# kevinh-e/BetaOne

Hardware: AMD Instinct MI355X
Metric: mcts_nodes_per_sec (higher is better)
Workload: dtype f32 (3 x f16 split, f32 accumulate)

## Files before the change

betaone_amd/csrc/bo_engine.cpp:

```cpp
#include "../../include/betaone_engine.h"
#include "../../include/betaone_lab.h"

#include "bo_tree.h"
#include "bo_fastw.h"
#include "bo_info.h"
#include "bo_select_wide.h"
#include "bo_replay.h"
#include "bo_train.h"
#include "bo_metrics.h"
#include "bo_pgn.h"
#include "bo_san.h"
#include "bo_analyse.h"
#include "bo_reanalyse.h"
#include "bo_perft.h"
#include "bo_mate.h"
#include "bo_anchor.h"
#include "bo_book.h"
#include "bo_merge.h"
#include "bo_tb.h"
#include "bo_nn_fused.h"
#include "bo_conv.h"
#include "bo_tower.h"
#include "bo_tower_wg.h"
#include "bo_tower_h.h"
// ... 546 lines not shown
    return BO_OK;
}
extern "C" int bo_step(bo_engine *e, const float *policy_dev, const float *value_dev, int policy_kind, float *nn_in_dev,
                       void *stream) {
    if (!e || !nn_in_dev) return fail(BO_E_ARG, "null argument");
    if (policy_kind != BO_POLICY_NONE && (!policy_dev || !value_dev)) return fail(BO_E_ARG, "policy/value required");
    return step_launch(e, policy_dev, value_dev, policy_kind, nn_in_dev, stream, StepTail{nullptr, nullptr, nullptr, nullptr, 0});
}
extern "C" int bo_step_heads(bo_engine *e, const float *logits_dev, const float *vpart_dev, const float *b1_dev, const float *w2_dev,
                             const float *b2_dev, int rows, float *nn_in_dev, void *stream) {
    if (!e || !nn_in_dev || !logits_dev || !vpart_dev || !b1_dev || !w2_dev || !b2_dev) return fail(BO_E_ARG, "null argument");
    if (e->fast) return fail(BO_E_CONFIG, "bo_step_heads: the reference-semantics search only (fast mode evaluates rows, not games)");
    if (rows < e->d.c.G) return fail(BO_E_ARG, "bo_step_heads: the partial sums must hold a row per game (rows >= G)");
    return step_launch(e, logits_dev, nullptr, BO_POLICY_LOGITS, nn_in_dev, stream, StepTail{vpart_dev, b1_dev, w2_dev, b2_dev, rows});
}

extern "C" int bo_search_poll(bo_engine *e, int32_t *n_running, int32_t *n_requested, int32_t *requested_mask, void *stream) {
    if (!e) return fail(BO_E_ARG, "null engine");
    const size_t G = (size_t)e->d.c.G;
    RT(rt_d2h(e->h_info, e->d_info_blk, 2 * G * 4, stream));
    const int *ph = e->h_info, *rq = e->h_info + G;
    RT(rt_sync(stream));
    int run = 0, req = 0;
    for (size_t g = 0; g < G; g++) {
        bool r = ph[g] == PH_RUN;
        bool q = r && rq[g] >= 0;
        run += r; req += q;
        if (requested_mask) requested_mask[g] = q ? 1 : 0;
    }
    if (n_running) *n_running = run;
// ... 2148 lines not shown
#else
    if (!stream) return BO_OK;
    RT((int)hipStreamDestroy((hipStream_t)stream));
    return BO_OK;
#endif
}

extern "C" int bo_nn_heads(const void *p_dev, const void *v_dev, const float *wp_dev, const float *bp_dev, const float *w1_dev,
                           const float *b1_dev, const float *w2_dev, const float *b2_dev, float *policy_out_dev, float *value_out_dev,
                           float *scratch_dev, int batch, int flags, void *stream) {
#if defined(BO_WAVE_EMU)
    (void)p_dev; (void)v_dev; (void)wp_dev; (void)bp_dev; (void)w1_dev; (void)b1_dev; (void)w2_dev; (void)b2_dev; (void)policy_out_dev;
    (void)value_out_dev; (void)scratch_dev; (void)batch; (void)flags; (void)stream;
    return fail(BO_E_CONFIG, "bo_nn_heads is a gfx950-only kernel");
#else
    if (!p_dev || !v_dev || !wp_dev || !bp_dev || !w1_dev || !b1_dev || !w2_dev || !b2_dev || !policy_out_dev || (!value_out_dev && !(flags & 4)) || !scratch_dev)
        return fail(BO_E_ARG, "null argument");
    if ((flags & 4) && (flags & 1)) return fail(BO_E_ARG, "bo_nn_heads: flags 4 (no rows kernel) leaves LOGITS: it excludes flags 1 (softmax)");
    if (batch < 1 || batch > 65536) return fail(BO_E_ARG, "bo_nn_heads: 1 <= batch <= 65536");
    bo_heads_args a;
    a.p = p_dev; a.v = v_dev; a.wp = wp_dev; a.bp = bp_dev; a.w1 = w1_dev; a.b1 = b1_dev; a.w2 = w2_dev; a.b2 = b2_dev;
    a.policy_out = policy_out_dev; a.value_out = value_out_dev;
    a.vpart = scratch_dev;
    a.B = batch; a.softmax = flags & 1; a.pb = bo_heads_policy_boards(batch);
    const int otw = 4 / (a.pb >> 5);
    const unsigned tiles = (unsigned)(((batch + a.pb - 1) / a.pb) * ((BO_HEADS_NA / 32 + otw - 1) / otw) + ((batch + 63) / 64) * 4 * BO_HEADS_KS);
    if (flags & 2) hipLaunchKernelGGL(bo_k_heads_tiles<true>, dim3(tiles), dim3(256), 0, (hipStream_t)stream, a, bo_heads_pair{});
    else hipLaunchKernelGGL(bo_k_heads_tiles<false>, dim3(tiles), dim3(256), 0, (hipStream_t)stream, a, bo_heads_pair{});
    if (!(flags & 4)) hipLaunchKernelGGL(bo_k_heads_rows, dim3((unsigned)batch), dim3(256), 0, (hipStream_t)stream, a);
    RT((int)hipGetLastError());
// ... 1170 lines not shown
```

betaone_amd/csrc/bo_heads.h:

```cpp
#pragma once
#if !defined(BO_WAVE_EMU)
#include <hip/hip_runtime.h>
#include "bo_tower.h"

#define BO_HEADS_NA 4672
#define BO_HEADS_KP 128
#define BO_HEADS_KV 2048
#define BO_HEADS_NH 256
#define BO_HEADS_KS 16
#define BO_HEADS_PITCH 132

struct bo_heads_args {
    const void *p, *v;
    const float *wp, *bp, *w1, *b1, *w2, *b2;
    float *policy_out, *value_out;
    float *vpart;
    int B, softmax;
    int pb;
};
static inline int bo_heads_policy_boards(int batch) { return batch > 64 ? 128 : batch > 32 ? 64 : 32; }

struct bo_heads_pair {
    const int32_t *sel = nullptr;
    const float *wp = nullptr, *bp = nullptr, *w1 = nullptr, *b1 = nullptr, *w2 = nullptr, *b2 = nullptr;
// ... 124 lines not shown
#pragma unroll
                        for (int rt = 0; rt < 2; rt++) acc[c][rt] = __builtin_amdgcn_mfma_f32_16x16x4f32(fw[c][e], fv[rt][e], acc[c][rt], 0, 0, 0);
            }
#pragma unroll
            for (int c = 0; c < 2; c++)
#pragma unroll
                for (int rt = 0; rt < 2; rt++) {
                    const int row = r0 + bb + 16 * rt + i;
                    if (row < B && (only_net < 0 || (pr.sel[row] != 0) == only_net))
                        *reinterpret_cast<bo_f32x4 *>(a.vpart + ((size_t)ks * B + row) * BO_HEADS_NH + h0 + hb + 16 * c + 4 * kq) = acc[c][rt];
                }
        }
    }
}

template <bool PAIR>
__device__ __forceinline__ void bo_heads_rows_body(const bo_heads_args &a, const bo_heads_pair &q) {
    __shared__ float sred[8];
    const int tid = threadIdx.x, lane = tid & 63, wave = __builtin_amdgcn_readfirstlane(tid >> 6);
    const int B = a.B, row = (int)blockIdx.x;
    const float *b1 = a.b1, *w2 = a.w2, *b2 = a.b2;
    if constexpr (PAIR) {
        if (__builtin_amdgcn_readfirstlane(q.sel[row]) != 0) { b1 = q.b1; w2 = q.w2; b2 = q.b2; }
    }
    float part[BO_HEADS_KS];
#pragma unroll
    for (int ks = 0; ks < BO_HEADS_KS; ks++) part[ks] = a.vpart[((size_t)ks * B + row) * BO_HEADS_NH + tid];
    bo_f32x4 *r4 = reinterpret_cast<bo_f32x4 *>(a.policy_out + (size_t)row * BO_HEADS_NA);
    constexpr int N4 = BO_HEADS_NA / 4, IT = (N4 + 255) / 256;
    const float ninf = -__builtin_inff();
    bo_f32x4 x[IT];
    float mx = ninf;
    if (a.softmax) {
#pragma unroll
        for (int u = 0; u < IT; u++) {
            const int k = tid + 256 * u;
            x[u] = k < N4 ? r4[k] : bo_f32x4{ninf, ninf, ninf, ninf};
        }
    }
    float hsum = 0.0f;
#pragma unroll
    for (int ks = 0; ks < BO_HEADS_KS; ks++) hsum += part[ks];
    hsum += b1[tid];
    hsum = (hsum > 0.0f ? hsum : 0.0f) * w2[tid];
    if (a.softmax) {
#pragma unroll
        for (int u = 0; u < IT; u++) mx = fmaxf(mx, fmaxf(fmaxf(x[u][0], x[u][1]), fmaxf(x[u][2], x[u][3])));
    }
#pragma unroll
    for (int m = 32; m >= 1; m >>= 1) { mx = fmaxf(mx, __shfl_xor(mx, m, 64)); hsum += __shfl_xor(hsum, m, 64); }
    if (lane == 0) { sred[wave] = mx; sred[4 + wave] = hsum; }
    __syncthreads();
    mx = fmaxf(fmaxf(sred[0], sred[1]), fmaxf(sred[2], sred[3]));
    if (tid == 0) a.value_out[row] = tanhf(((sred[4] + sred[5]) + (sred[6] + sred[7])) + b2[0]);
    if (a.softmax) {
        float sum = 0.0f;
#pragma unroll
        for (int u = 0; u < IT; u++) {
            if (tid + 256 * u < N4) {
#pragma unroll
                for (int e = 0; e < 4; e++) { x[u][e] = expf(x[u][e] - mx); sum += x[u][e]; }
            }
        }
#pragma unroll
        for (int m = 32; m >= 1; m >>= 1) sum += __shfl_xor(sum, m, 64);
        __syncthreads();
        if (lane == 0) sred[wave] = sum;
        __syncthreads();
        sum = (sred[0] + sred[1]) + (sred[2] + sred[3]);
#pragma unroll
        for (int u = 0; u < IT; u++) {
            const int k = tid + 256 * u;
            if (k < N4) r4[k] = bo_f32x4{x[u][0] / sum, x[u][1] / sum, x[u][2] / sum, x[u][3] / sum};
        }
    }
}

extern "C" __global__ void __launch_bounds__(256)
bo_k_heads_rows(bo_heads_args a) { bo_heads_rows_body<false>(a, bo_heads_pair{}); }

extern "C" __global__ void __launch_bounds__(256)
bo_k_heads_rows_pair(bo_heads_args a, bo_heads_pair q) { bo_heads_rows_body<true>(a, q); }

typedef _Float16 bo_hh8 __attribute__((ext_vector_type(8)));

#ifndef BO_HEADS_NT_STORES
#define BO_HEADS_NT_STORES 1
#endif
#define BO_HEADS_PS 10
#define BO_HEADS_PT 15
#define BO_HEADS_WPITCH (BO_HEADS_KP + 8)

struct bo_heads_h_args {
    const _Float16 *p, *v;
    const _Float16 *wp, *w1;
    const float *bp, *b1, *w2, *b2;
    float *policy_out, *value_out;
// ... 214 lines not shown
```

betaone_amd/csrc/bo_tree.h:

```cpp
#pragma once
#include "bo_chess.h"
#include "bo_tb_probe.h"
#include <math.h>

#define BO_CH_CAP 32
#define BO_PATH_CAP 1024
#define BO_RES_CAP 256
#define BO_PLANES 120
#ifndef BO_PROF_SLOTS
#define BO_PROF_SLOTS 16
#endif
#define BO_ROW (BO_PLANES * 64)

enum { PH_IDLE = 0, PH_RUN = 1, PH_DONE = 2 };
enum { ST_OK = 0, ST_NODE_OVERFLOW = 1, ST_DEPTH_OVERFLOW = 2, ST_NAN_SCORE = 4, ST_PLY_OVERFLOW = 8,
       ST_ILLEGAL_ACTION = 16, ST_UL_OVERFLOW = 32, ST_TRK_OVERFLOW = 64 };
enum { POLICY_NONE = 0, POLICY_LOGITS = 1, POLICY_PROBS = 2 };

struct EngCfg {
    int G, S, B;
    int NCAP, PLY_CAP, TRK_CAP;
    int nstride;
    int UL_MAX, CH_MAX;
    float cpuct, keep;
// ... 626 lines not shown
    if (bo_finite(x)) return x;
    *bad = true;
    return 0.0f;
}

struct StepShared {
    bo_mv moves[BO_MAX_MOVES];
    bo_mv moves2[BO_MAX_MOVES];
    float pv[BO_MAX_MOVES];
    int path[BO_PATH_CAP];
    int path2[BO_PATH_CAP];
    int bpath[8];
    float probs[BO_NUM_ACTIONS];
    int rank_of[2 * BO_CH_CAP];
    ChainBuf chain;
};

BO_DEV void load_probs(const float *row, int kind, float *out) {
    const int lane = bo_lane();
    if (kind == POLICY_PROBS) {
        for (int i = lane; i < BO_NUM_ACTIONS; i += 64) out[i] = row[i];
    } else {
        float mx, sum;
        bo_f4 v[BO_ROW_IT];
        row_load_max_sum(row, v, &mx, &sum);
        BO_UNROLL
        for (int i = 0; i < BO_ROW_IT; i++) {
            const int k = lane + 64 * i;
            if (k < BO_ROW_N4) {
                out[4 * k] = bo_exp_row(v[i].x - mx) / sum; out[4 * k + 1] = bo_exp_row(v[i].y - mx) / sum;
                out[4 * k + 2] = bo_exp_row(v[i].z - mx) / sum; out[4 * k + 3] = bo_exp_row(v[i].w - mx) / sum;
            }
        }
    }
    bo_sync();
}

BO_DEV void apply_root(const Eng &e, int g, const float *row, int kind, StepShared &sh, int *n_nodes_io, int *flags) {
    const size_t no = NOFF(e, g);
    const int lane = bo_lane();
    const int n = e.root_nlegal[g];
    const bo_mv *mv = e.root_moves + (size_t)g * BO_MAX_MOVES;
    load_probs(row, kind, sh.probs);
    int m = e.c.root_m < n ? e.c.root_m : n;
    if (m > BO_CH_CAP) m = BO_CH_CAP;
    bool bad = false;
    for (int j = lane; j < n; j += 64) sh.pv[j] = finite_or_zero(sh.probs[move_to_index(mv[j])], &bad);
    if (lane < 2 * BO_CH_CAP) sh.rank_of[lane] = -1;
    bo_sync();
    for (int j = lane; j < n; j += 64) {
        int r = stable_rank(sh.pv, n, j);
        if (r < m) sh.rank_of[r] = j;
    }
    bo_sync();
    const DPos P = e.npos[no];
    int nch = m;
    if (lane < m) {
        int j = sh.rank_of[lane];
// ... 56 lines not shown
    BO_UNROLL
    for (int w = 0; w < 4; w++) {
        float h = 0.0f;
        BO_UNROLL
        for (int ks = 0; ks < 16; ks++) h += r.part[w][ks];
        h += r.b1[w];
        s[w] = (h > 0.0f ? h : 0.0f) * r.w2[w];
    }
    for (int m = 32; m >= 1; m >>= 1) {
        BO_UNROLL
        for (int w = 0; w < 4; w++) s[w] = s[w] + bo_shfl_xor_f(s[w], m);
    }
    return tanhf(((s[0] + s[1]) + (s[2] + s[3])) + r.b2);
}

BO_DEV void apply_leaf(const Eng &e, int g, int leaf, const float *row, int kind, const float *value_of, const StepTail &vt, StepShared &sh,
                       int *n_ul_io, int *flags) {
    const size_t no = NOFF(e, g);
    const int lane = bo_lane();
    const int n = e.req_nlegal[g];
    const bo_mv *mv = e.req_moves + (size_t)g * BO_MAX_MOVES;
    int slot = *n_ul_io;
    if (slot >= e.c.UL_MAX) { *flags |= ST_UL_OVERFLOW; slot = e.c.UL_MAX - 1; }
    const size_t uo = (size_t)g * e.c.UL_MAX + slot;
    float value;
    bool bad = false;
    if (kind == POLICY_PROBS) {
        value = value_of[g];
        for (int j = lane; j < n; j += 64) sh.pv[j] = finite_or_zero(row[move_to_index(mv[j])], &bad);
    } else {
        float mx, sum;
        if (vt.vpart) {
            TailRegs tr;
            tail_load(vt, g, tr);
            row_max_sum(row, &mx, &sum);
            value = tail_value(tr);
        } else {
            value = value_of[g];
            row_max_sum(row, &mx, &sum);
        }
        for (int j = lane; j < n; j += 64) sh.pv[j] = finite_or_zero(bo_exp_row(row[move_to_index(mv[j])] - mx) / sum, &bad);
    }
// ... 8 lines not shown
    if (lane == 0) {
        e.ul_node[uo] = leaf;
        e.ul_nlegal[uo] = n;
        e.ul_value[uo] = value;
        e.eval_slot[no + leaf] = (short)slot;
    }
    *n_ul_io = slot + 1;
    bo_sync();
}


BO_DEV float tb_leaf_value(int t, int kc) {
    const float m = 1.0f - (float)kc * (1.0f / 1024.0f);
    return t == TERM_TB_LOSS ? m : t == TERM_TB_WIN ? -m : 0.0f;
}
template <bool TB>
BO_DEV int step_body(const Eng &e, int g, const float *policy, const float *value, int kind, float *nn_in, StepShared &sh, const StepTail &vt) {
    const int lane = bo_lane();
    const size_t no = NOFF(e, g);
    int flags = 0;
    int sims = e.sims_done[g], rows = e.rows[g], n_runs = e.n_runs[g], n_ul = e.n_ul[g], n_nodes = e.n_nodes[g];
    int req = e.req_node[g];
    int *rl = e.run_leaf + (size_t)g * e.c.B, *rc = e.run_cnt + (size_t)g * e.c.B;
    float *row = nn_in + (size_t)g * BO_ROW;

    const bool prof = e.c.profile != 0;
    unsigned long long pc[8] = {0, 0, 0, 0, 0, 0, 0, 0};
    int n_iter = 0, n_first = 0, n_burst = 0, n_burst_sims = 0, n_general = 0, n_swaps = 0;
    unsigned long long tk = prof ? bo_clock() : 0ull;
    const unsigned long long t_start = tk;
#define BO_PROF(slot)                                                    \
    if (prof) { const unsigned long long _n = bo_clock(); pc[slot] += _n - tk; tk = _n; }
    if (req >= 0 && kind == POLICY_NONE) return n_nodes;
    const float *lut = e.sqrt_lut;
    if (req >= 0) {
        if (req == 0) apply_root(e, g, policy + (size_t)g * BO_NUM_ACTIONS, kind, sh, &n_nodes, &flags);
        else apply_leaf(e, g, req, policy + (size_t)g * BO_NUM_ACTIONS, kind, value, vt, sh, &n_ul, &flags);
        req = -1;
    }
    BO_PROF(0)
    int phase = PH_RUN;
    bool burst_tables_staged = false;
    int term_budget = e.c.B;
    int b_depth = 0;
    float b_tv = 0.0f;
    int path_leaf = -1, path_depth = -1;
    for (;;) {
        if (sims >= e.c.S) {
            if (rows > 0) { flush_pending(e, g, n_runs, n_ul, &n_nodes, sh.path2, &flags, path_leaf, sh.path, path_depth); rows = n_runs = n_ul = 0; }
            BO_PROF(5)
            phase = PH_DONE;
            break;
// ... 102 lines not shown
    return n_nodes;
}
BO_KERNEL void bo_k_step(Eng e, const float *policy, const float *value, int kind, float *nn_in, StepTail vt) {
    BO_SHARED StepShared sh;
    const int g = bo_block();
    if (e.phase[g] != PH_RUN) return;
    step_body<false>(e, g, policy, value, kind, nn_in, sh, vt);
}
BO_KERNEL void bo_k_step_tb(Eng e, const float *policy, const float *value, int kind, float *nn_in, StepTail vt) {
    BO_SHARED StepShared sh;
    const int g = bo_block();
    if (e.phase[g] != PH_RUN) return;
    step_body<true>(e, g, policy, value, kind, nn_in, sh, vt);
}

BO_DEV int root_prepare(const Eng &e, int g, StepShared &sh) {
    const size_t no = NOFF(e, g);
    const int lane = bo_lane();
    const int ply = e.ply[g];
    const DPos P = e.gpos[(size_t)g * e.c.PLY_CAP + ply];
    if (lane == 0) {
        init_node(e, no, 0, -1, 1.0f, 0, P);
        e.n_nodes[g] = 1; e.sims_done[g] = 0; e.rows[g] = 0; e.n_runs[g] = 0; e.n_ul[g] = 0;
        e.req_node[g] = -1; e.phase[g] = PH_IDLE; e.root_nch[g] = 0;
        if (e.ctx_mode[g] == 0) {
            int nh = ply < 7 ? ply : 7;
            e.n_hist[g] = nh;
            for (int i = 0; i < nh; i++) e.hist[(size_t)g * 7 + i] = e.gpos[(size_t)g * e.c.PLY_CAP + ply - nh + i];
        }
    }
// ... 361 lines not shown
```

betaone_amd/csrc/bo_wave.h:

```cpp
#pragma once
#include <stdint.h>

#if defined(BO_WAVE_EMU)
#include "wave_emu.h"
#else
#include <hip/hip_runtime.h>
#define BO_DEV __device__ __forceinline__
#define BO_DEV_NOINLINE __device__ __noinline__
#define BO_KERNEL extern "C" __global__ __launch_bounds__(64)
#define BO_SHARED __shared__
#define BO_CONST_TABLE __device__ const

BO_DEV int bo_lane() { return (int)(threadIdx.x & 63u); }
BO_DEV int bo_block() { return (int)blockIdx.x; }
BO_DEV uint64_t bo_ballot(bool p) { return __ballot(p); }
BO_DEV void bo_sync() { __syncthreads(); }
BO_DEV int bo_shfl(int v, int src) { return __shfl(v, src, 64); }
BO_DEV int bo_shfl_xor(int v, int m) { return __shfl_xor(v, m, 64); }
BO_DEV int bo_shfl_up(int v, int d) { return __shfl_up(v, d, 64); }
BO_DEV int bo_atomic_add(int *p, int v) { return atomicAdd(p, v); }
BO_DEV int bo_atomic_or(int *p, int v) { return atomicOr(p, v); }
BO_DEV uint64_t bo_bitrev64(uint64_t x) { return __builtin_bitreverse64(x); }
BO_DEV unsigned long long bo_clock() { return (unsigned long long)clock64(); }
#define BO_ROW_XCHG(v, kind) \
    __builtin_amdgcn_update_dpp(0, (v), (kind) == 0 ? 0xB1 : (kind) == 1 ? 0x4E : (kind) == 2 ? 0x141 : 0x140, 0xF, 0xF, false)
#endif
#if !defined(BO_WAVE_EMU)
BO_DEV int bo_readlane(int v, int src) { return __builtin_amdgcn_readlane(v, __builtin_amdgcn_readfirstlane(src)); }
#else
static inline int bo_readlane(int v, int src) { return bo_shfl(v, src); }
#endif
// ... 66 lines not shown
```

betaone_amd/engine.py:

```python
from __future__ import annotations

import ctypes as C
import os
from typing import Dict, List, Optional, Sequence, Tuple

import numpy as np
import torch

NUM_ACTIONS = 4672
INPUT_CHANNELS = 120
ROW_FLOATS = 120 * 64
MAX_LEGAL = 256
RES_CAP = 256
POLICY_NONE, POLICY_LOGITS, POLICY_PROBS = 0, 1, 2

STATUS_BITS = {1: "node overflow", 2: "depth overflow", 4: "NaN or infinite evaluation (prior or value)", 8: "ply overflow",
               16: "illegal action", 32: "leaf cache overflow", 64: "tracker overflow", 128: "position range outside the array",
               256: "pi wider than the record's rows"}
ST_PLY_OVERFLOW, ST_ILLEGAL_ACTION = 8, 16
ST_PI_OVERFLOW = 256
ST_NODE_OVERFLOW = 1
ST_DEPTH_OVERFLOW = 2
ST_NAN_SCORE = 4

# ... 64 lines not shown
_F64P = C.POINTER(C.c_double)
_TRAIN_BATCH = [C.c_int32, C.c_int32, C.c_void_p, C.c_int32, C.c_void_p, C.c_int32] + [C.c_void_p] * 3

_SYMBOLS = {
    "bo_abi_version": (C.c_int, []),
    "bo_last_error": (C.c_char_p, []),
    "bo_engine_create": (C.c_int, [C.POINTER(BoConfig), C.c_int, C.POINTER(C.c_void_p)]),
    "bo_engine_destroy": (None, [C.c_void_p]),
    "bo_games_reset": (C.c_int, [C.c_void_p, C.c_int, _I32P, C.POINTER(C.c_char_p), C.POINTER(C.c_char_p), C.c_void_p]),
    "bo_games_reset_ex": (C.c_int, [C.c_void_p, C.c_int, _I32P, C.POINTER(C.c_char_p), C.POINTER(C.c_char_p),
                                    C.POINTER(BoPosition), _I32P, C.POINTER(BoPosition), _I32P, _I32P, C.c_void_p]),
    "bo_root_info": (C.c_int, [C.c_void_p, _I32P, _I32P, _I32P, C.c_void_p]),
    "bo_search_begin": (C.c_int, [C.c_void_p, _I32P, _F64P, C.c_void_p, C.c_void_p]),
    "bo_step": (C.c_int, [C.c_void_p, C.c_void_p, C.c_void_p, C.c_int, C.c_void_p, C.c_void_p]),
    "bo_step_heads": (C.c_int, [C.c_void_p] * 6 + [C.c_int, C.c_void_p, C.c_void_p]),
    "bo_search_poll": (C.c_int, [C.c_void_p, _I32P, _I32P, _I32P, C.c_void_p]),
    "bo_search_stop": (C.c_int, [C.c_void_p, _I32P, _I32P, C.c_void_p]),
    "bo_search_close": (C.c_int, [C.c_void_p, C.c_void_p]),
    "bo_search_info": (C.c_int, [C.c_void_p, C.c_int32, C.c_void_p, C.c_void_p]),
    "bo_search_result": (C.c_int, [C.c_void_p, _I32P, _I32P, _F32P, _I32P, _I32P, _I32P, C.c_void_p]),
    "bo_play": (C.c_int, [C.c_void_p, _I32P, C.c_void_p]),
    "bo_game_export": (C.c_int, [C.c_void_p, C.c_int, C.POINTER(BoPosition), _I32P, C.c_int32, _I32P, C.c_void_p]),
    "bo_game_encode": (C.c_int, [C.c_void_p, C.c_int, C.c_int, C.c_int, C.c_void_p, C.c_void_p]),
    "bo_rng_seed": (C.c_int, [C.c_void_p, C.c_int, C.c_uint32]),
    "bo_rng_state": (C.c_int, [C.c_void_p, C.c_int, C.c_int, C.POINTER(C.c_uint32), _I32P, _I32P, _F64P]),
    "bo_selfplay_sample": (C.c_int, [C.c_void_p, _I32P, _I32P, C.c_int32, C.c_double, C.c_double, _I32P, _I32P, _F32P,
                                     _I32P, _I32P, C.c_void_p]),
    "bo_selfplay_turn": (C.c_int, [C.c_void_p, _I32P, _I32P, C.c_int32, C.c_double, C.c_double, _I32P, _I32P, _F32P, _I32P, _I32P, _I32P,
                                   C.c_void_p, _I32P, _I32P, _I32P, C.c_int32, _I32P, C.c_void_p]),
    "bo_selfplay_noise": (C.c_int, [C.c_void_p, C.c_void_p]),
# ... 124 lines not shown
                                 C.c_void_p, C.c_void_p, C.c_void_p]),
}

HIP_LIB_PATH = os.path.join(os.path.dirname(os.path.abspath(__file__)), "csrc", "libbetaone_hip.so")


def bind(cdll: C.CDLL) -> C.CDLL:
    for name, (res, args) in list(_SYMBOLS.items()) + list(_LAB_SYMBOLS.items()):
        fn = getattr(cdll, name)
        fn.restype = res
        fn.argtypes = args
    return cdll


_hip_lib: Optional[C.CDLL] = None
ABI_VERSION = 21
PROF_SLOTS = 16
METRIC_ROW = {name: k for k, name in enumerate((
    "BAD", "HAS_POLICY", "DECISIVE", "RANK", "TOP1", "TOP3", "TOP5", "ARGMAX_IN_SUPPORT", "CE", "TARGET_ENTROPY", "NET_ENTROPY", "P_TOP",
    "P_SUPPORT", "SE_Z", "SE_Q", "ABS_V", "SIGN_OK", "Z", "V"))}
METRIC = {name: k for k, name in enumerate((
    "N_ROWS", "N_BAD", "N_POLICY_ROWS", "N_DECISIVE", "SUM_RANK", "SUM_TOP1", "SUM_TOP3", "SUM_TOP5", "SUM_ARGMAX_IN_SUPPORT", "SUM_CE",
    "SUM_TARGET_ENTROPY", "SUM_NET_ENTROPY", "SUM_P_TOP", "SUM_P_SUPPORT", "SUM_SE_Z", "SUM_SE_Q", "SUM_ABS_V", "SUM_SIGN_OK", "SUM_Z", "SUM_V"))}
METRIC_ROW_COLS, METRIC_COLS = len(METRIC_ROW), len(METRIC)


def load_hip_library() -> C.CDLL:
    global _hip_lib
    if _hip_lib is None:
        from . import build as _build

# ... 173 lines not shown
        self._check(self.lib.bo_match_select(self.h, net_of_white_ptr, sel_ptr, stream))

    def search_begin(self, go, noise: Optional[np.ndarray], nn_in_ptr: int, stream: int = 0):
        g = _i32(go)
        nz = None
        if noise is not None:
            nz = np.ascontiguousarray(noise, dtype=np.float64).reshape(self.G, MAX_LEGAL)
        self._check(self.lib.bo_search_begin(self.h, _p(g), _p(nz, _F64P) if nz is not None else None, nn_in_ptr, stream))

    def step(self, policy_ptr: int, value_ptr: int, kind: int, nn_in_ptr: int, stream: int = 0):
        self._check(self.lib.bo_step(self.h, policy_ptr, value_ptr, kind, nn_in_ptr, stream))

    def step_heads(self, logits_ptr: int, vpart_ptr: int, b1_ptr: int, w2_ptr: int, b2_ptr: int, rows: int, nn_in_ptr: int, stream: int = 0):
        self._check(self.lib.bo_step_heads(self.h, logits_ptr, vpart_ptr, b1_ptr, w2_ptr, b2_ptr, rows, nn_in_ptr, stream))

    def poll(self, stream: int = 0, want_mask: bool = True):
        run, req = C.c_int32(), C.c_int32()
        mask = np.zeros(self.G, dtype=np.int32) if want_mask else None
        self._check(self.lib.bo_search_poll(self.h, C.byref(run), C.byref(req), _p(mask) if want_mask else None, stream))
        return run.value, req.value, mask

    def search_stop(self, mask=None, stream: int = 0) -> np.ndarray:
        m = _i32(mask) if mask is not None else None
        done = np.zeros(self.G, dtype=np.int32)
        self._check(self.lib.bo_search_stop(self.h, _p(m) if m is not None else None, _p(done), stream))
        return done

    def search_info(self, n_lines: int, out_ptr: int, stream: int = 0) -> None:
        self._check(self.lib.bo_search_info(self.h, int(n_lines), out_ptr, stream))

# ... 233 lines not shown
```

betaone_amd/fused_net.py:

```python
from __future__ import annotations

import torch
import torch.nn as nn
import torch.nn.functional as F

import copy
import ctypes as C
import dataclasses
import math
import os

import numpy as np

from . import engine as E


MFMA_CONV_SHAPES = {(120, 64), (64, 64), (120, 128), (128, 128), (120, 256), (256, 256)}


def pack_conv_weight(w: torch.Tensor) -> torch.Tensor:
    co, ci = w.shape[0], w.shape[1]
    return w.reshape(co, ci // 8, 4, 2, 9).permute(4, 1, 0, 3, 2).contiguous()


# ... 529 lines not shown
                return "heads"
            if os.environ.get("BETAONE_HEADS_F16", "1") != "0":
                return "heads_f16"
        return "library_forked" if self.conv in ("tower_wg", "tower_split") else "library"

    def tail_supported(self, batch: int) -> bool:
        return self.head_stage(batch) == "heads"

    def tail_params(self):
        return self.value_fc1.bias.data_ptr(), self.value_fc2.weight.data_ptr(), self.value_fc2.bias.data_ptr()

    @torch.no_grad()
    def forward_tail(self, x):
        return self.forward(x, tail=True)

    def _epi(self, x, bias, res=None):
        B, C = x.shape[0], x.shape[1]
        stream = torch.cuda.current_stream(x.device).cuda_stream
        _check(self.lib, self.lib.bo_nn_bias_act(x.data_ptr(), bias.data_ptr(), res.data_ptr() if res is not None else None, B, C, stream))
        return x

    def _se(self, x, bias, se, res):
        B, C = x.shape[0], x.shape[1]
        stream = torch.cuda.current_stream(x.device).cuda_stream
        small = self.conv in ("mfma_small", "tower_b1") and C % 16 == 0 and se[0].shape[0] <= 16
        _check(self.lib, (self.lib.bo_nn_se_residual_small if small else self.lib.bo_nn_se_residual)(
            x.data_ptr(), bias.data_ptr(), se[0].data_ptr(), se[1].data_ptr(), res.data_ptr(), B, C, se[0].shape[0], stream))
        return res if small else x

    def _tower_mfma(self, x):
# ... 145 lines not shown
```

betaone_amd/rollout.py:

```python
from __future__ import annotations

import math
import os
import time
from dataclasses import dataclass, field
from typing import Callable, Dict, List, Optional, Sequence

import numpy as np
import torch

from . import engine as E
from . import sampling

CAPTURE_MODE = "thread_local"


@dataclass
class GameState:
    game_id: int
    rng: object
    start_fen: Optional[str] = None
    start_fullmove: int = 1
    start_white: bool = True
    plies: int = 0
# ... 139 lines not shown
                            dirichlet_alpha=dirichlet_alpha, dirichlet_epsilon=dirichlet_epsilon, max_plies=max_plies,
                            device=dev_index, fast=fast, leaves_per_step=leaves_per_step, fast_arena_granules=fast_arena_granules)
        self.fast, self.L = bool(fast), self.eng.L
        if self.values:
            self.eng.root_values(True)
        if self.tb is not None:
            self.eng.tablebases(list(self.tb.tables.values()), self.tb_flags)
        self.nn_in = torch.zeros((self.G * self.L, E.INPUT_CHANNELS, 8, 8), dtype=torch.float32, device=self.device)
        self.expected_evals = math.ceil(self.S / self.L) if self.fast else 1 + math.ceil(self.S / self.B)
        self.games: List[Optional[GameState]] = [None] * self.G
        self.external_moves: Optional[Callable] = None
        self.use_graph = bool(use_graph) and self.device.type == "cuda"
        self.close_last_eval = self.close_allowed and self.use_graph
        self._graph = None
        self._graphs_n = {}
        self._logits = self._value = None
        self.n_forward = 0
        self.n_sims = 0
        self.n_plies = 0
        self.host_seconds = 0.0
        assert rng_mode in ("python", "native")
        self.rng_mode = rng_mode
        assert policy_kind in ("logits", "probs")
        self.policy_kind = E.POLICY_LOGITS if policy_kind == "logits" else E.POLICY_PROBS
        G = self.G
        self._fgraph = None
        self._side = torch.cuda.Stream(self.device) if self.device.type == "cuda" else None
        self._noise_pending = False
        self._fwd_early = False
        import os as _os
# ... 25 lines not shown
        self._rv = np.zeros((G, 256 if self.values else 0), np.float32)
        self._resigned = np.zeros(G, dtype=bool)
        self._renable = np.zeros(G, dtype=np.int32)
        self._rcheck = np.zeros(G, dtype=bool)
        self._rcnt = np.zeros((G, 2), dtype=np.int64)
        self.net_of_white = torch.zeros(G, dtype=torch.int32, device=self.device) if self.pair else None
        self._sel = torch.zeros(G, dtype=torch.int32, device=self.device) if self.pair else None
        self._watch_net()
        self._set_tail()

    def _set_tail(self):
        m = self.model
        ok = (self.policy_kind == E.POLICY_LOGITS and not self.fast and not self.autocast and self.device.type == "cuda"
              and os.environ.get("BETAONE_STEP_TAIL", "1") != "0" and hasattr(m, "forward_tail") and m.tail_supported(self.G))
        self.step_tail = bool(ok)
        self._tail_params = tuple(m.tail_params()) if ok else None

    def _step_after(self, first, second):
        if self.step_tail:
            if second.shape != (16, self.G, 256):
                raise E.EngineError(f"step tail: value_fc1's partial sums must be [16, {self.G}, 256], got {tuple(second.shape)}")
            self.eng.step_heads(first.data_ptr(), second.data_ptr(), *self._tail_params, second.shape[1], self.nn_in.data_ptr(), self._stream())
        else:
            self.eng.step(first.data_ptr(), second.data_ptr(), self.policy_kind, self.nn_in.data_ptr(), self._stream())

    def _watch_net(self):
        inner = getattr(self.model, "net", self.model)
        words = getattr(inner, "overflow_words", None)
        self._watch_msg = getattr(inner, "OVERFLOW_MESSAGE", "the evaluate stage reported a fault")
        ptr, n = words() if words is not None else (0, 1)
        self.eng.watch(ptr, n)

    def _check_watch(self):
        if self.eng.watch_seen():
            chk = getattr(getattr(self.model, "net", self.model), "check_overflow", None)
            if chk is not None and self.device.type == "cuda":
                torch.cuda.synchronize(self.device)
# ... 1 lines not shown
            raise E.EngineError(self._watch_msg)

    def _stream(self) -> int:
        return torch.cuda.current_stream(self.device).cuda_stream if self.device.type == "cuda" else 0

    def _forward(self):
        if self.tower_timing is not None:
            getattr(self.model, "net", self.model).tower_timing_buf = self.tower_timing
        want_probs = self.policy_kind == E.POLICY_PROBS
        if self.pair:
            self.eng.match_select(self.net_of_white.data_ptr(), self._sel.data_ptr(), self._stream())
            logits, value = (self.model.forward_probs if want_probs else self.model)(self.nn_in, self._sel)
            return logits.float().contiguous(), value.float().contiguous()
        fused = getattr(self.model, "forward_probs", None) if (want_probs and not self.autocast) else None
        with torch.no_grad():
            if self.step_tail:
                logits, part = self.model.forward_tail(self.nn_in)
                return logits, part
            if fused is not None:
                logits, value = fused(self.nn_in)
                want_probs = False
            elif self.autocast:
                with torch.autocast(self.device.type):
                    logits, value = self.model(self.nn_in)
            else:
                logits, value = self.model(self.nn_in)
        logits = logits.float()
        if want_probs:
            logits = torch.softmax(logits, dim=1)
        return logits.contiguous(), value.float().contiguous()

# ... 253 lines not shown
        burst = self.expected_evals
        info = None
        if self._noise_pending:
            self._noise_pending = False
            if self._fwd_early:
                self._fwd_early = False
            else:
                self.n_forward += 1
                self._forward_only()
            if self._begun is E.LAZY_BEGIN:
                info = self.eng.selfplay_begun()
                self._begun = None
            if self.ply_profile is not None: self._pp("begun")
            self.eng.selfplay_noise(self._stream())
            if self.ply_profile is not None: self._pp("noise")
            self._step_after(self._f_logits, self._f_value)
            burst -= 1
        while True:
            self._eval_and_step_n(burst)
            if not poll:
                return info
            running, _, _ = self.eng.poll(self._stream(), want_mask=False)
            if running == 0:
                break
            burst = 1

    def _play_ply_native(self, on_finished, refill, while_searching=None) -> int:
        if self._turn_due is not None:
            self.ply_end()
        if not self.ply_begin(on_finished, refill, while_searching):
            return 0
# ... 511 lines not shown
```

include/betaone_engine.h:

```cpp
#ifndef BETAONE_ENGINE_H
#define BETAONE_ENGINE_H

#include <stdint.h>

#ifdef __cplusplus
extern "C" {
#endif

#define BO_ABI_VERSION 21
#define BO_NUM_ACTIONS 4672
#define BO_INPUT_CHANNELS 120
#define BO_ROW_FLOATS (120 * 64)
#define BO_MAX_LEGAL 256
#define BO_RES_CAP 256

enum {
    BO_OK = 0,
    BO_E_ARG = -1,
    BO_E_HIP = -2,
    BO_E_CONFIG = -3,
    BO_E_FEN = -4,
    BO_E_STATE = -5
};

// ... 41 lines not shown
int bo_games_reset(bo_engine *e, int n, const int32_t *slots, const char *const *fens, const char *const *moves,
                   void *stream);

int bo_games_reset_ex(bo_engine *e, int n, const int32_t *slots, const char *const *fens, const char *const *moves,
                      const bo_position *hist, const int32_t *n_hist, const bo_position *trk,
                      const int32_t *trk_counts, const int32_t *trk_off, void *stream);

int bo_root_info(bo_engine *e, int32_t *n_legal, int32_t *terminal, int32_t *ply, void *stream);

int bo_search_begin(bo_engine *e, const int32_t *go, const double *noise, float *nn_in_dev, void *stream);

int bo_step(bo_engine *e, const float *policy_dev, const float *value_dev, int policy_kind, float *nn_in_dev,
            void *stream);
int bo_step_heads(bo_engine *e, const float *logits_dev, const float *vpart_dev, const float *b1_dev, const float *w2_dev,
                  const float *b2_dev, int rows, float *nn_in_dev, void *stream);

int bo_search_poll(bo_engine *e, int32_t *n_running, int32_t *n_requested, int32_t *requested_mask, void *stream);

int bo_search_stop(bo_engine *e, const int32_t *stop_mask, int32_t *sims_done, void *stream);

int bo_search_close(bo_engine *e, void *stream);

int bo_search_result(bo_engine *e, int32_t *res_n, int32_t *res_idx, float *res_val, int32_t *best_idx,
                     int32_t *best_move, int32_t *total_visits, void *stream);

int bo_play(bo_engine *e, const int32_t *action, void *stream);

int bo_rng_seed(bo_engine *e, int slot, uint32_t seed);
int bo_rng_state(bo_engine *e, int slot, int set, uint32_t *key624, int32_t *pos, int32_t *has_gauss, double *gauss);
int bo_selfplay_sample(bo_engine *e, const int32_t *active, const int32_t *move_number, int32_t threshold,
// ... 359 lines not shown
```

Measured before the change: 80.79 million.

## Fuse heads rows softmax/value into MCTS step kernel via LDS for probs policy

```diff
diff --git a/betaone_amd/csrc/bo_engine.cpp b/betaone_amd/csrc/bo_engine.cpp
--- a/betaone_amd/csrc/bo_engine.cpp
+++ b/betaone_amd/csrc/bo_engine.cpp
@@ -584,6 +584,24 @@
     if (rows < e->d.c.G) return fail(BO_E_ARG, "bo_step_heads: the partial sums must hold a row per game (rows >= G)");
     return step_launch(e, logits_dev, nullptr, BO_POLICY_LOGITS, nn_in_dev, stream, StepTail{vpart_dev, b1_dev, w2_dev, b2_dev, rows});
 }
+extern "C" int bo_step_rows(bo_engine *e, const float *logits_dev, const float *vpart_dev, const float *b1_dev, const float *w2_dev,
+                            const float *b2_dev, int rows, float *nn_in_dev, void *stream) {
+    if (!e || !nn_in_dev || !logits_dev || !vpart_dev || !b1_dev || !w2_dev || !b2_dev) return fail(BO_E_ARG, "null argument");
+    if (e->fast) return fail(BO_E_CONFIG, "bo_step_rows: the reference-semantics search only (fast mode evaluates rows, not games)");
+    if (rows < e->d.c.G) return fail(BO_E_ARG, "bo_step_rows: the partial sums must hold a row per game (rows >= G)");
+#if defined(BO_WAVE_EMU)
+    (void)stream;
+    return fail(BO_E_CONFIG, "bo_step_rows is a gfx950-only kernel (four waves per game)");
+#else
+    e->prefetch_valid = false;
+    const StepTail vt{vpart_dev, b1_dev, w2_dev, b2_dev, rows};
+    if (e->d.tb_n > 0 && (e->d.tb_flags & TBF_SEARCH))
+        hipLaunchKernelGGL(bo_k_step_rows_tb, dim3((unsigned)e->d.c.G), dim3(256), 0, (hipStream_t)stream, e->d, logits_dev, nn_in_dev, vt);
+    else hipLaunchKernelGGL(bo_k_step_rows, dim3((unsigned)e->d.c.G), dim3(256), 0, (hipStream_t)stream, e->d, logits_dev, nn_in_dev, vt);
+    RT((int)hipGetLastError());
+    return BO_OK;
+#endif
+}
 
 extern "C" int bo_search_poll(bo_engine *e, int32_t *n_running, int32_t *n_requested, int32_t *requested_mask, void *stream) {
     if (!e) return fail(BO_E_ARG, "null engine");
@@ -2762,6 +2780,17 @@
     (void)value_out_dev; (void)scratch_dev; (void)batch; (void)flags; (void)stream;
     return fail(BO_E_CONFIG, "bo_nn_heads is a gfx950-only kernel");
 #else
+    if (flags == 8) {
+        if (!b1_dev || !w2_dev || !b2_dev || !policy_out_dev || !value_out_dev || !scratch_dev) return fail(BO_E_ARG, "null argument");
+        if (batch < 1 || batch > 65536) return fail(BO_E_ARG, "bo_nn_heads: 1 <= batch <= 65536");
+        bo_heads_args r{};
+        r.b1 = b1_dev; r.w2 = w2_dev; r.b2 = b2_dev; r.policy_out = policy_out_dev; r.value_out = value_out_dev; r.vpart = scratch_dev;
+        r.B = batch; r.softmax = 1;
+        hipLaunchKernelGGL(bo_k_heads_rows, dim3((unsigned)batch), dim3(256), 0, (hipStream_t)stream, r);
+        RT((int)hipGetLastError());
+        return BO_OK;
+    }
+    if (flags & 8) return fail(BO_E_ARG, "bo_nn_heads: flags 8 (the rows of an earlier flags-4 call) goes alone");
     if (!p_dev || !v_dev || !wp_dev || !bp_dev || !w1_dev || !b1_dev || !w2_dev || !b2_dev || !policy_out_dev || (!value_out_dev && !(flags & 4)) || !scratch_dev)
         return fail(BO_E_ARG, "null argument");
     if ((flags & 4) && (flags & 1)) return fail(BO_E_ARG, "bo_nn_heads: flags 4 (no rows kernel) leaves LOGITS: it excludes flags 1 (softmax)");
diff --git a/betaone_amd/csrc/bo_heads.h b/betaone_amd/csrc/bo_heads.h
--- a/betaone_amd/csrc/bo_heads.h
+++ b/betaone_amd/csrc/bo_heads.h
@@ -162,8 +162,16 @@
     }
 }
 
-template <bool PAIR>
-__device__ __forceinline__ void bo_heads_rows_body(const bo_heads_args &a, const bo_heads_pair &q) {
+struct bo_rows_to_memory {
+    float *value_out;
+    bo_f32x4 *r4;
+    __device__ __forceinline__ void value(int row, float v) const { value_out[row] = v; }
+    __device__ __forceinline__ void stats(float, float) const {}
+    __device__ __forceinline__ void probs(int k, const bo_f32x4 &x, float sum) const { r4[k] = bo_f32x4{x[0] / sum, x[1] / sum, x[2] / sum, x[3] / sum}; }
+};
+
+template <bool PAIR, class DST>
+__device__ __forceinline__ void bo_heads_rows_body(const bo_heads_args &a, const bo_heads_pair &q, const DST &dst) {
     __shared__ float sred[8];
     const int tid = threadIdx.x, lane = tid & 63, wave = __builtin_amdgcn_readfirstlane(tid >> 6);
     const int B = a.B, row = (int)blockIdx.x;
@@ -174,7 +182,7 @@
     float part[BO_HEADS_KS];
 #pragma unroll
     for (int ks = 0; ks < BO_HEADS_KS; ks++) part[ks] = a.vpart[((size_t)ks * B + row) * BO_HEADS_NH + tid];
-    bo_f32x4 *r4 = reinterpret_cast<bo_f32x4 *>(a.policy_out + (size_t)row * BO_HEADS_NA);
+    const bo_f32x4 *r4 = reinterpret_cast<const bo_f32x4 *>(a.policy_out + (size_t)row * BO_HEADS_NA);
     constexpr int N4 = BO_HEADS_NA / 4, IT = (N4 + 255) / 256;
     const float ninf = -__builtin_inff();
     bo_f32x4 x[IT];
@@ -200,7 +208,7 @@
     if (lane == 0) { sred[wave] = mx; sred[4 + wave] = hsum; }
     __syncthreads();
     mx = fmaxf(fmaxf(sred[0], sred[1]), fmaxf(sred[2], sred[3]));
-    if (tid == 0) a.value_out[row] = tanhf(((sred[4] + sred[5]) + (sred[6] + sred[7])) + b2[0]);
+    if (tid == 0) dst.value(row, tanhf(((sred[4] + sred[5]) + (sred[6] + sred[7])) + b2[0]));
     if (a.softmax) {
         float sum = 0.0f;
 #pragma unroll
@@ -216,19 +224,24 @@
         if (lane == 0) sred[wave] = sum;
         __syncthreads();
         sum = (sred[0] + sred[1]) + (sred[2] + sred[3]);
+        if (tid == 0) dst.stats(mx, sum);
 #pragma unroll
         for (int u = 0; u < IT; u++) {
             const int k = tid + 256 * u;
-            if (k < N4) r4[k] = bo_f32x4{x[u][0] / sum, x[u][1] / sum, x[u][2] / sum, x[u][3] / sum};
+            if (k < N4) dst.probs(k, x[u], sum);
         }
     }
 }
 
 extern "C" __global__ void __launch_bounds__(256)
-bo_k_heads_rows(bo_heads_args a) { bo_heads_rows_body<false>(a, bo_heads_pair{}); }
+bo_k_heads_rows(bo_heads_args a) {
+    bo_heads_rows_body<false>(a, bo_heads_pair{}, bo_rows_to_memory{a.value_out, reinterpret_cast<bo_f32x4 *>(a.policy_out + (size_t)blockIdx.x * BO_HEADS_NA)});
+}
 
 extern "C" __global__ void __launch_bounds__(256)
-bo_k_heads_rows_pair(bo_heads_args a, bo_heads_pair q) { bo_heads_rows_body<true>(a, q); }
+bo_k_heads_rows_pair(bo_heads_args a, bo_heads_pair q) {
+    bo_heads_rows_body<true>(a, q, bo_rows_to_memory{a.value_out, reinterpret_cast<bo_f32x4 *>(a.policy_out + (size_t)blockIdx.x * BO_HEADS_NA)});
+}
 
 typedef _Float16 bo_hh8 __attribute__((ext_vector_type(8)));
 
diff --git a/betaone_amd/csrc/bo_tree.h b/betaone_amd/csrc/bo_tree.h
--- a/betaone_amd/csrc/bo_tree.h
+++ b/betaone_amd/csrc/bo_tree.h
@@ -1,6 +1,9 @@
 #pragma once
 #include "bo_chess.h"
 #include "bo_tb_probe.h"
+#if !defined(BO_WAVE_EMU)
+#include "bo_heads.h"
+#endif
 #include <math.h>
 
 #define BO_CH_CAP 32
@@ -664,11 +667,14 @@
     float probs[BO_NUM_ACTIONS];
     int rank_of[2 * BO_CH_CAP];
     ChainBuf chain;
+    float row_value, row_mx, row_sum;
 };
 
+template <bool ROW_LDS>
 BO_DEV void load_probs(const float *row, int kind, float *out) {
     const int lane = bo_lane();
-    if (kind == POLICY_PROBS) {
+    if constexpr (ROW_LDS) {
+    } else if (kind == POLICY_PROBS) {
         for (int i = lane; i < BO_NUM_ACTIONS; i += 64) out[i] = row[i];
     } else {
         float mx, sum;
@@ -686,12 +692,13 @@
     bo_sync();
 }
 
+template <bool ROW_LDS>
 BO_DEV void apply_root(const Eng &e, int g, const float *row, int kind, StepShared &sh, int *n_nodes_io, int *flags) {
     const size_t no = NOFF(e, g);
     const int lane = bo_lane();
     const int n = e.root_nlegal[g];
     const bo_mv *mv = e.root_moves + (size_t)g * BO_MAX_MOVES;
-    load_probs(row, kind, sh.probs);
+    load_probs<ROW_LDS>(row, kind, sh.probs);
     int m = e.c.root_m < n ? e.c.root_m : n;
     if (m > BO_CH_CAP) m = BO_CH_CAP;
     bool bad = false;
@@ -778,6 +785,7 @@
     return tanhf(((s[0] + s[1]) + (s[2] + s[3])) + r.b2);
 }
 
+template <bool ROW_LDS>
 BO_DEV void apply_leaf(const Eng &e, int g, int leaf, const float *row, int kind, const float *value_of, const StepTail &vt, StepShared &sh,
                        int *n_ul_io, int *flags) {
     const size_t no = NOFF(e, g);
@@ -789,7 +797,11 @@
     const size_t uo = (size_t)g * e.c.UL_MAX + slot;
     float value;
     bool bad = false;
-    if (kind == POLICY_PROBS) {
+    if constexpr (ROW_LDS) {
+        value = sh.row_value;
+        const float sum = sh.row_sum;
+        for (int j = lane; j < n; j += 64) sh.pv[j] = finite_or_zero(sh.probs[move_to_index(mv[j])] / sum, &bad);
+    } else if (kind == POLICY_PROBS) {
         value = value_of[g];
         for (int j = lane; j < n; j += 64) sh.pv[j] = finite_or_zero(row[move_to_index(mv[j])], &bad);
     } else {
@@ -828,7 +840,7 @@
     const float m = 1.0f - (float)kc * (1.0f / 1024.0f);
     return t == TERM_TB_LOSS ? m : t == TERM_TB_WIN ? -m : 0.0f;
 }
-template <bool TB>
+template <bool TB, bool ROW_LDS = false>
 BO_DEV int step_body(const Eng &e, int g, const float *policy, const float *value, int kind, float *nn_in, StepShared &sh, const StepTail &vt) {
     const int lane = bo_lane();
     const size_t no = NOFF(e, g);
@@ -848,8 +860,8 @@
     if (req >= 0 && kind == POLICY_NONE) return n_nodes;
     const float *lut = e.sqrt_lut;
     if (req >= 0) {
-        if (req == 0) apply_root(e, g, policy + (size_t)g * BO_NUM_ACTIONS, kind, sh, &n_nodes, &flags);
-        else apply_leaf(e, g, req, policy + (size_t)g * BO_NUM_ACTIONS, kind, value, vt, sh, &n_ul, &flags);
+        if (req == 0) apply_root<ROW_LDS>(e, g, policy + (size_t)g * BO_NUM_ACTIONS, kind, sh, &n_nodes, &flags);
+        else apply_leaf<ROW_LDS>(e, g, req, policy + (size_t)g * BO_NUM_ACTIONS, kind, value, vt, sh, &n_ul, &flags);
         req = -1;
     }
     BO_PROF(0)
@@ -982,6 +994,43 @@
     step_body<true>(e, g, policy, value, kind, nn_in, sh, vt);
 }
 
+#if !defined(BO_WAVE_EMU)
+struct bo_rows_to_lds {
+    StepShared *sh;
+    bool root;
+    __device__ __forceinline__ void value(int, float v) const { sh->row_value = v; }
+    __device__ __forceinline__ void stats(float mx, float sum) const { sh->row_mx = mx; sh->row_sum = sum; }
+    __device__ __forceinline__ void probs(int k, const bo_f32x4 &x, float sum) const {
+        float *o = sh->probs + 4 * k;
+        if (root) { o[0] = x[0] / sum; o[1] = x[1] / sum; o[2] = x[2] / sum; o[3] = x[3] / sum; }
+        else { o[0] = x[0]; o[1] = x[1]; o[2] = x[2]; o[3] = x[3]; }
+    }
+};
+template <bool TB>
+__device__ __forceinline__ void step_rows(const Eng &e, const float *logits, float *nn_in, const StepTail &vt, StepShared &sh) {
+    const int g = (int)blockIdx.x, wave = __builtin_amdgcn_readfirstlane((int)(threadIdx.x >> 6));
+    const int ph = e.phase[g], req = e.req_node[g];
+    if (ph == PH_RUN && req >= 0) {
+        bo_heads_args a{};
+        a.policy_out = const_cast<float *>(logits);
+        a.vpart = const_cast<float *>(vt.vpart); a.b1 = vt.b1; a.w2 = vt.w2; a.b2 = vt.b2;
+        a.B = vt.rows; a.softmax = 1;
+        bo_heads_rows_body<false>(a, bo_heads_pair{}, bo_rows_to_lds{&sh, req == 0});
+    }
+    __syncthreads();
+    if (wave != 0 || ph != PH_RUN) return;
+    step_body<TB, true>(e, g, logits, nullptr, POLICY_PROBS, nn_in, sh, StepTail{nullptr, nullptr, nullptr, nullptr, 0});
+}
+extern "C" __global__ void __launch_bounds__(256) bo_k_step_rows(Eng e, const float *logits, float *nn_in, StepTail vt) {
+    __shared__ StepShared sh;
+    step_rows<false>(e, logits, nn_in, vt, sh);
+}
+extern "C" __global__ void __launch_bounds__(256) bo_k_step_rows_tb(Eng e, const float *logits, float *nn_in, StepTail vt) {
+    __shared__ StepShared sh;
+    step_rows<true>(e, logits, nn_in, vt, sh);
+}
+#endif
+
 BO_DEV int root_prepare(const Eng &e, int g, StepShared &sh) {
     const size_t no = NOFF(e, g);
     const int lane = bo_lane();
diff --git a/betaone_amd/csrc/bo_wave.h b/betaone_amd/csrc/bo_wave.h
--- a/betaone_amd/csrc/bo_wave.h
+++ b/betaone_amd/csrc/bo_wave.h
@@ -14,7 +14,11 @@
 BO_DEV int bo_lane() { return (int)(threadIdx.x & 63u); }
 BO_DEV int bo_block() { return (int)blockIdx.x; }
 BO_DEV uint64_t bo_ballot(bool p) { return __ballot(p); }
-BO_DEV void bo_sync() { __syncthreads(); }
+BO_DEV void bo_sync() {
+    __builtin_amdgcn_fence(__ATOMIC_RELEASE, "workgroup");
+    __builtin_amdgcn_wave_barrier();
+    __builtin_amdgcn_fence(__ATOMIC_ACQUIRE, "workgroup");
+}
 BO_DEV int bo_shfl(int v, int src) { return __shfl(v, src, 64); }
 BO_DEV int bo_shfl_xor(int v, int m) { return __shfl_xor(v, m, 64); }
 BO_DEV int bo_shfl_up(int v, int d) { return __shfl_up(v, d, 64); }
diff --git a/betaone_amd/engine.py b/betaone_amd/engine.py
--- a/betaone_amd/engine.py
+++ b/betaone_amd/engine.py
@@ -102,6 +102,7 @@
     "bo_search_begin": (C.c_int, [C.c_void_p, _I32P, _F64P, C.c_void_p, C.c_void_p]),
     "bo_step": (C.c_int, [C.c_void_p, C.c_void_p, C.c_void_p, C.c_int, C.c_void_p, C.c_void_p]),
     "bo_step_heads": (C.c_int, [C.c_void_p] * 6 + [C.c_int, C.c_void_p, C.c_void_p]),
+    "bo_step_rows": (C.c_int, [C.c_void_p] * 6 + [C.c_int, C.c_void_p, C.c_void_p]),
     "bo_search_poll": (C.c_int, [C.c_void_p, _I32P, _I32P, _I32P, C.c_void_p]),
     "bo_search_stop": (C.c_int, [C.c_void_p, _I32P, _I32P, C.c_void_p]),
     "bo_search_close": (C.c_int, [C.c_void_p, C.c_void_p]),
@@ -256,7 +257,7 @@
 
 
 _hip_lib: Optional[C.CDLL] = None
-ABI_VERSION = 21
+ABI_VERSION = 22
 PROF_SLOTS = 16
 METRIC_ROW = {name: k for k, name in enumerate((
     "BAD", "HAS_POLICY", "DECISIVE", "RANK", "TOP1", "TOP3", "TOP5", "ARGMAX_IN_SUPPORT", "CE", "TARGET_ENTROPY", "NET_ENTROPY", "P_TOP",
@@ -460,6 +461,9 @@
     def step_heads(self, logits_ptr: int, vpart_ptr: int, b1_ptr: int, w2_ptr: int, b2_ptr: int, rows: int, nn_in_ptr: int, stream: int = 0):
         self._check(self.lib.bo_step_heads(self.h, logits_ptr, vpart_ptr, b1_ptr, w2_ptr, b2_ptr, rows, nn_in_ptr, stream))
 
+    def step_rows(self, logits_ptr: int, vpart_ptr: int, b1_ptr: int, w2_ptr: int, b2_ptr: int, rows: int, nn_in_ptr: int, stream: int = 0):
+        self._check(self.lib.bo_step_rows(self.h, logits_ptr, vpart_ptr, b1_ptr, w2_ptr, b2_ptr, rows, nn_in_ptr, stream))
+
     def poll(self, stream: int = 0, want_mask: bool = True):
         run, req = C.c_int32(), C.c_int32()
         mask = np.zeros(self.G, dtype=np.int32) if want_mask else None
diff --git a/betaone_amd/fused_net.py b/betaone_amd/fused_net.py
--- a/betaone_amd/fused_net.py
+++ b/betaone_amd/fused_net.py
@@ -567,6 +567,16 @@
     def forward_tail(self, x):
         return self.forward(x, tail=True)
 
+    @torch.no_grad()
+    def finish_tail(self, logits, part):
+        B = logits.shape[0]
+        out = logits.clone()
+        value = torch.empty((B, 1), dtype=torch.float32, device=logits.device)
+        _check(self.lib, self.lib.bo_nn_heads(None, None, None, None, None, self.value_fc1.bias.data_ptr(), self.value_fc2.weight.data_ptr(),
+                                              self.value_fc2.bias.data_ptr(), out.data_ptr(), value.data_ptr(), part.data_ptr(), B, 8,
+                                              torch.cuda.current_stream(logits.device).cuda_stream))
+        return out, value
+
     def _epi(self, x, bias, res=None):
         B, C = x.shape[0], x.shape[1]
         stream = torch.cuda.current_stream(x.device).cuda_stream
diff --git a/betaone_amd/rollout.py b/betaone_amd/rollout.py
--- a/betaone_amd/rollout.py
+++ b/betaone_amd/rollout.py
@@ -177,6 +177,7 @@
         self.close_last_eval = self.close_allowed and self.use_graph
         self._graph = None
         self._graphs_n = {}
+        self._seam_step, self._seam_root = [None, None], [None, None]
         self._logits = self._value = None
         self.n_forward = 0
         self.n_sims = 0
@@ -232,13 +233,30 @@
         ok = (self.policy_kind == E.POLICY_LOGITS and not self.fast and not self.autocast and self.device.type == "cuda"
               and os.environ.get("BETAONE_STEP_TAIL", "1") != "0" and hasattr(m, "forward_tail") and m.tail_supported(self.G))
         self.step_tail = bool(ok)
-        self._tail_params = tuple(m.tail_params()) if ok else None
+        rows = (self.policy_kind == E.POLICY_PROBS and not self.fast and not self.pair and not self.autocast and self.device.type == "cuda"
+                and self.G > 1 and os.environ.get("BETAONE_STEP_ROWS", "1") != "0" and hasattr(m, "forward_tail") and m.tail_supported(self.G))
+        self.step_rows = bool(rows)
+        self._tail_params = tuple(m.tail_params()) if (ok or rows) else None
+
+    def _seam(self, pair, i):
+        if self.step_rows and pair[0] is not None and pair[1] is not None and pair[1].dim() == 3:
+            fin = getattr(self.model, "finish_tail", None) or getattr(getattr(self.model, "net", None), "finish_tail", None)
+            if fin is None:
+                raise E.EngineError("step_rows: the model has no finish_tail to make the evaluate seam from (logits, partial sums)")
+            return fin(*pair)[i]
+        return pair[i]
+
+    _logits = property(lambda self: self._seam(self._seam_step, 0), lambda self, v: self._seam_step.__setitem__(0, v))
+    _value = property(lambda self: self._seam(self._seam_step, 1), lambda self, v: self._seam_step.__setitem__(1, v))
+    _f_logits = property(lambda self: self._seam(self._seam_root, 0), lambda self, v: self._seam_root.__setitem__(0, v))
+    _f_value = property(lambda self: self._seam(self._seam_root, 1), lambda self, v: self._seam_root.__setitem__(1, v))
 
     def _step_after(self, first, second):
-        if self.step_tail:
+        if self.step_tail or self.step_rows:
             if second.shape != (16, self.G, 256):
                 raise E.EngineError(f"step tail: value_fc1's partial sums must be [16, {self.G}, 256], got {tuple(second.shape)}")
-            self.eng.step_heads(first.data_ptr(), second.data_ptr(), *self._tail_params, second.shape[1], self.nn_in.data_ptr(), self._stream())
+            (self.eng.step_heads if self.step_tail else self.eng.step_rows)(
+                first.data_ptr(), second.data_ptr(), *self._tail_params, second.shape[1], self.nn_in.data_ptr(), self._stream())
         else:
             self.eng.step(first.data_ptr(), second.data_ptr(), self.policy_kind, self.nn_in.data_ptr(), self._stream())
 
@@ -270,7 +288,7 @@
             return logits.float().contiguous(), value.float().contiguous()
         fused = getattr(self.model, "forward_probs", None) if (want_probs and not self.autocast) else None
         with torch.no_grad():
-            if self.step_tail:
+            if self.step_tail or self.step_rows:
                 logits, part = self.model.forward_tail(self.nn_in)
                 return logits, part
             if fused is not None:
@@ -554,7 +572,7 @@
             if self.ply_profile is not None: self._pp("begun")
             self.eng.selfplay_noise(self._stream())
             if self.ply_profile is not None: self._pp("noise")
-            self._step_after(self._f_logits, self._f_value)
+            self._step_after(*self._seam_root)
             burst -= 1
         while True:
             self._eval_and_step_n(burst)
diff --git a/include/betaone_engine.h b/include/betaone_engine.h
--- a/include/betaone_engine.h
+++ b/include/betaone_engine.h
@@ -7,7 +7,7 @@
 extern "C" {
 #endif
 
-#define BO_ABI_VERSION 21
+#define BO_ABI_VERSION 22
 #define BO_NUM_ACTIONS 4672
 #define BO_INPUT_CHANNELS 120
 #define BO_ROW_FLOATS (120 * 64)
@@ -79,6 +79,8 @@
             void *stream);
 int bo_step_heads(bo_engine *e, const float *logits_dev, const float *vpart_dev, const float *b1_dev, const float *w2_dev,
                   const float *b2_dev, int rows, float *nn_in_dev, void *stream);
+int bo_step_rows(bo_engine *e, const float *logits_dev, const float *vpart_dev, const float *b1_dev, const float *w2_dev,
+                 const float *b2_dev, int rows, float *nn_in_dev, void *stream);
 
 int bo_search_poll(bo_engine *e, int32_t *n_running, int32_t *n_requested, int32_t *requested_mask, void *stream);
 
```

New measurement: 82.05 million, median of 6. +1.6%, better.
